# sloup/hessgpu

Hardware: AMD Instinct MI355X
Metric: Mpixels/s end-to-end (pyramid->descriptor), 1920x1080 (higher is better)
Workload: dtype f32; 1 GPU; 1920x1080 synthetic blobs (tests/fixtures.py), default octaves/DoG levels, top-K=4096 [configs[1]]; pipelined_contexts_per_gpu=6, streams_and_copier_threads_per_node=6, descriptor_order=pixel, distinct_images_per_gpu=8, input=u8 luminance resident in HBM; results delivered to host memory

## Files before the change

hessgpu_amd/csrc/k_feature.hip:

```cpp
#include <algorithm>
#include <cstdlib>
#include <type_traits>

#include "hess_dev.h"
#include "hess_devmath.h"

namespace hess {

namespace {

constexpr double kPI = 3.14159265358979323846;

__device__ __forceinline__ float rl(float v, int lane) {
  return __uint_as_float(__builtin_amdgcn_readlane(__float_as_uint(v), lane));
}
__device__ __forceinline__ int rli(int v, int lane) { return __builtin_amdgcn_readlane(v, lane); }

__device__ __forceinline__ void level_of(const Geom& g, int li, int* o, int* l) {
  *o = li / g.dog;
  *l = li - (*o) * g.dog + 1;
}


__device__ __forceinline__ int block_scan1(int a, int* total, int* lds) {
  const int lane = threadIdx.x & 63, wv = threadIdx.x >> 6, nw = blockDim.x >> 6;
  int ia = a;
#pragma unroll
  for (int d = 1; d < 64; d <<= 1) {
    int na = __shfl_up(ia, d);
    if (lane >= d) ia += na;
  }
  __syncthreads();
  if (lane == 63) lds[wv] = ia;
  __syncthreads();
  int oa = 0, sa = 0;
  for (int k = 0; k < nw; k++) {
    if (k < wv) oa += lds[k];
    sa += lds[k];
  }
  *total = sa;
  return oa + ia - a;
}

struct FeatScan {
  LimitParams lp;
  int multi;
  int* foffset;
  int* fsrc;
  int* feat_total;
  int* feat_first;
  int cap_feat;
  int* overflow;
  int* img_base;
  int* host_small;
};

__device__ __forceinline__ int wave_inclusive_scan(int v) {
  v += __builtin_amdgcn_update_dpp(0, v, 0x111 , 0xf, 0xf, true);
  v += __builtin_amdgcn_update_dpp(0, v, 0x112 , 0xf, 0xf, true);
  v += __builtin_amdgcn_update_dpp(0, v, 0x114 , 0xf, 0xf, true);
  v += __builtin_amdgcn_update_dpp(0, v, 0x118 , 0xf, 0xf, true);
  v += __builtin_amdgcn_update_dpp(0, v, 0x142 , 0xa, 0xf, false);
  v += __builtin_amdgcn_update_dpp(0, v, 0x143 , 0xc, 0xf, false);
  return v;
}

__device__ __forceinline__ void feature_scan_image(const Geom& g, const FeatScan& fs, const RawKey* list, const int* list_total,
                                                   int cap_list, const int* ocount, int b, int nimg, int chunk, int nchunk) {
  const LimitParams& lp = fs.lp;
  const int multi = fs.multi, cap_feat = fs.cap_feat;
  int* const foffset = fs.foffset; int* const fsrc = fs.fsrc; int* const feat_total = fs.feat_total;
  int* const feat_first = fs.feat_first; int* const overflow = fs.overflow; int* const img_base = fs.img_base;
  int* const host_small = fs.host_small;
  __shared__ int lds[64];
  __shared__ int lc[kMaxOct * kMaxDog];
  __shared__ int carry;
  const int tid = threadIdx.x, NTH = blockDim.x;
  const int n = list_total[b];
  const bool need_levels = multi && lp.threshold > 0 && lp.method != 3;
  if (need_levels) nchunk = 1;
  if (chunk >= nchunk) return;
  const int clen = (((n + nchunk - 1) / nchunk) + 1023) & ~1023;
  const int c0 = min(n, chunk * clen), c1 = min(n, c0 + clen);
  const int lane = tid & 63, wv = tid >> 6, nwv = NTH >> 6;
  for (int i = tid; i < g.nlev; i += NTH) lc[i] = 0;
  {
    int before = multi ? 0 : c0;
    if (multi && c0 > 0) {
      int part = 0;
      for (int k = tid; k < c0; k += NTH) part += ocount[(long long)b * cap_list + k];
      part = wave_inclusive_scan(part);
      if (lane == 63) lds[wv] = part;
      __syncthreads();
      for (int w = 0; w < nwv; w++) before += lds[w];
      __syncthreads();
    }
    if (tid == 0) carry = before;
  }
  __syncthreads();
  constexpr int FC = 16;
  for (int base = c0; base < c1; base += NTH * FC) {
    const int npass = min(c1 - base, NTH * FC);
    const int fc = (npass + NTH - 1) / NTH;
    int cc[FC], ex[FC], tot[FC], wsum = 0;
#pragma unroll
    for (int u = 0; u < FC; u++) {
      const int k = (wv * fc + u) * 64 + lane;
      const bool in = u < fc && k < npass;
      const long long at = (long long)b * cap_list + base + (in ? k : 0);
      cc[u] = in ? (multi ? ocount[at] : 1) : 0;
      const int inc = wave_inclusive_scan(cc[u]);
      ex[u] = inc - cc[u];
      tot[u] = __builtin_amdgcn_readlane(inc, 63);
      wsum += tot[u];
      if (need_levels && tot[u]) {
        const int lv = in ? list[at].level_index : 0;
        const int lv0 = __builtin_amdgcn_readfirstlane(lv);
        if (__builtin_amdgcn_ballot_w64(cc[u] != 0 && lv != lv0) == 0) {
          if (lane == 0) atomicAdd(&lc[lv0], tot[u]);
        } else if (cc[u]) {
          atomicAdd(&lc[lv], cc[u]);
        }
      }
    }
    if (lane == 0) lds[wv] = wsum;
    __syncthreads();
    int run = carry, ptot = 0;
    for (int w = 0; w < nwv; w++) {
      const int t = lds[w];
      run += w < wv ? t : 0;
      ptot += t;
    }
#pragma unroll
    for (int u = 0; u < FC; u++) {
      const int k = (wv * fc + u) * 64 + lane;
      if (u < fc && k < npass) {
        const int off = run + ex[u];
        foffset[(long long)b * cap_list + base + k] = off;
        for (int q = 0; q < cc[u]; q++)
          if (off + q < cap_feat) fsrc[(long long)b * cap_feat + off + q] = (base + k) * 4 + q;
      }
      run += tot[u];
    }
    __syncthreads();
    if (tid == 0) carry += ptot;
    __syncthreads();
  }
  if (chunk != nchunk - 1) return;
  if (tid == 0) {
    int total = carry, first = 0;
    if (multi && lp.threshold > 0 && lp.method != 3) {
      if (lp.method == 2) {
        int i = 0, nf = 0;
        for (; (nf < lp.threshold) && (i < g.nlev); ++i) nf += lc[i];
        if (nf < total) total = nf;
      } else {
        int i = 0;
        while (i < g.nlev && (total - lc[i]) > lp.threshold) { total -= lc[i]; first += lc[i]; i++; }
      }
    }
    if (first + total > cap_feat) { atomicMax(overflow + 1, first + total); total = cap_feat > first ? cap_feat - first : 0; }
    feat_total[b] = total;
    feat_first[b] = first;
    __threadfence();
    if (atomicAdd(overflow + 8, 1) == nimg - 1) {
      __threadfence();
      int acc = 0;
      for (int i = 0; i < nimg; i++) {
        img_base[i] = acc;
        if (host_small) host_small[i] = acc;
        acc += __hip_atomic_load(feat_total + i, __ATOMIC_RELAXED, __HIP_MEMORY_SCOPE_AGENT);
      }
      img_base[nimg] = acc;
      if (host_small) {
        host_small[nimg] = acc;
        for (int i = 0; i < 4; i++)
          host_small[nimg + 1 + i] = __hip_atomic_load(overflow + i, __ATOMIC_RELAXED, __HIP_MEMORY_SCOPE_AGENT);
      }
    }
  }
}

__global__ __launch_bounds__(1024) void feature_scan_kernel(Geom g, FeatScan fs, const RawKey* list, const int* list_total,
                                                            int cap_list, const int* ocount) {
  feature_scan_image(g, fs, list, list_total, cap_list, ocount, (int)blockIdx.y, (int)gridDim.y, (int)blockIdx.x, (int)gridDim.x);
}


__device__ __forceinline__ void key_range(const KeyBinJob& j, int b, int* first, int* count) {
  const int f = min(max(j.first_count[2 * b], 0), j.total);
  *first = f;
  *count = min(max(j.first_count[2 * b + 1], 0), min(j.max_count, j.total - f));
}

__device__ __forceinline__ int key_fixed(float v, int n) {
  const double d = (double)(v * (float)(1 << n)) + ((v >= 0.0) ? 0.5 : -0.5);
  return (d > -2147483649.0 && d < 2147483648.0) ? (int)d : (int)0x80000000u;
}

__global__ __launch_bounds__(256) void key_level_kernel(KeyBinJob j) {
  const int b = blockIdx.y, i = blockIdx.x * 256 + threadIdx.x;
  int first, count;
  key_range(j, b, &first, &count);
  if (i >= count) return;
  const HostKeypoint key = j.keys[first + i];
  const float s = j.rect ? (key.s < key.o ? key.s : key.o) / 12.0f : key.s;
  const int given = j.levels ? j.levels[i] : -1;
  int m = 0, hits = 0;
  for (int lv = 0; lv < j.nlev; lv++) {
    const KeyLevel t = j.table[lv];
    float sigmak = s;
    if (given >= 0) {
      if (given != lv) continue;
      sigmak = t.level_sigma;
    }
    if (((sigmak >= t.sigma_min) && (sigmak < t.sigma_max)) || ((sigmak < t.sigma_min) && lv == 0) ||
        ((sigmak > t.sigma_max) && lv == j.nlev - 1)) {
      if (hits < 2) {
        m |= (lv + 1) << (16 * hits);
        atomicAdd(j.level_count + b * j.nlev + lv, 1);
      }
      hits++;
    }
  }
  j.member[(long long)b * j.max_count + i] = m;
  if (hits > 2) atomicMax(j.overflow, j.cap_list + 1);
}

__global__ __launch_bounds__(64) void key_bin_kernel(KeyBinJob j) {
  const int lv = blockIdx.x, b = blockIdx.y, lane = threadIdx.x;
  int first, count;
  key_range(j, b, &first, &count);
  int off = 0;
  for (int l = lane; l < lv; l += 64) off += j.level_count[b * j.nlev + l];
  off = __builtin_amdgcn_readlane(wave_inclusive_scan(off), 63);
  const int* const member = j.member + (long long)b * j.max_count;
  constexpr int KU = 4;
  for (int base = 0; base < count; base += 64 * KU) {
    int m[KU];
#pragma unroll
    for (int u = 0; u < KU; u++) {
      const int i = base + u * 64 + lane;
      m[u] = i < count ? member[i] : 0;
    }
#pragma unroll
    for (int u = 0; u < KU; u++) {
      const bool hit = (m[u] & 0xFFFF) == lv + 1 || (m[u] >> 16) == lv + 1;
      const unsigned long long hits = __builtin_amdgcn_ballot_w64(hit);
      const int pos = off + __builtin_popcountll(hits & ((1ull << lane) - 1ull));
      if (hit && pos < j.cap_list) {
        const long long at = (long long)b * j.cap_list + pos;
        const RawKey rk = {lv, 0, 0, 0u, 0.0f, 0.0f, 0.0f, 0u};
        j.list[at] = rk;
        j.kmap[at] = base + u * 64 + lane;
        if (j.host_kmap) j.host_kmap[at] = base + u * 64 + lane;
      }
      off += __builtin_popcountll(hits);
    }
  }
  if (lv == j.nlev - 1 && lane == 0) {
    if (off > j.cap_list) { atomicMax(j.overflow, off); off = j.cap_list; }
    j.list_total[b] = off;
  }
}

__global__ __launch_bounds__(256) void key_record_kernel(KeyBinJob j) {
  const int b = blockIdx.y, pos = blockIdx.x * 256 + threadIdx.x;
  int first, count;
  key_range(j, b, &first, &count);
  if (pos >= min(j.list_total[b], j.cap_list)) return;
  const long long at = (long long)b * j.cap_list + pos;
  const int i = min(max(j.kmap[at], 0), count - 1), lv = min(max(j.list[at].level_index, 0), j.nlev - 1);
  const KeyLevel t = j.table[lv];
  const HostKeypoint key = j.keys[first + i];
  const float fX = (key.x - j.origin) / t.octave_sigma + 0.5f;
  const float fY = (key.y - j.origin) / t.octave_sigma + 0.5f;
  const float fScale = key.s / t.octave_sigma;
  const float fOrientation = j.rect ? key.o / t.octave_sigma : (float)fmod(2.0 * kPI - (double)key.o, 2.0 * kPI);
  FRec r;
  r.x = (uint32_t)key_fixed(fX, 10) & 0x00FFFFFFu;
  r.y = (uint32_t)key_fixed(fY, 10) & 0x00FFFFFFu;
  r.z = (uint32_t)key_fixed(fScale, 8) & 0x0000FFFFu;
  r.w = __float_as_uint(fOrientation);
  j.recs[at] = r;
}


__device__ __forceinline__ float dm_expf_inrange(float x) {
  float n = rintf(x * 1.44269504088896341f);
  float r = fmaf(n, -0.693359375f, x);
  r = fmaf(n, 2.12194440e-4f, r);
  float z = r * r;
  float p = 1.9875691500E-4f;
  p = fmaf(p, r, 1.3981999507E-3f);
  p = fmaf(p, r, 8.3334519073E-3f);
  p = fmaf(p, r, 4.1665795894E-2f);
  p = fmaf(p, r, 1.6666665459E-1f);
  p = fmaf(p, r, 5.0000001201E-1f);
  p = fmaf(p, z, r);
  p = p + 1.0f;
  return __builtin_amdgcn_ldexpf(p, (int)n);
}


__global__ __launch_bounds__(256) void orientation_kernel(Geom g, OrientParams op, const RawKey* list,
                                                          const int* list_total, int cap_list, const float* got,
                                                          FRec* recs, int* ocount) {
  __shared__ __attribute__((aligned(8))) float2 orec[4][66];
  const int lane = threadIdx.x & 63;
  float2* const myrec = orec[threadIdx.x >> 6];
  __shared__ int osize[4][36];
  int* const mysize = osize[threadIdx.x >> 6];
  const int b = blockIdx.y;
  const int n = list_total[b];
  const int nwaves = gridDim.x * 4;
  const float ten_degree_per_radius = 5.7295779513082320876798154814105f;
  const float radius_per_ten_degrees = (float)(1.0 / 5.7295779513082320876798154814105);
  const float one_third = (float)(1.0 / 3.0);

  for (int i = blockIdx.x * 4 + (threadIdx.x >> 6); i < n; i += nwaves) {
    const RawKey rk = list[(long long)b * cap_list + i];
    int o, l;
    level_of(g, rk.level_index, &o, &l);
    const OctGeom& og = g.o[o];
    const float2* gp = reinterpret_cast<const float2*>(got) + og.got_off + ((long long)(l - 1) * g.B + b) * og.plane;
    const int width = og.wa, height = og.h;

    float kx = rk.col + 0.5f, ky = rk.row + 0.5f, kz = op.level_sigma[l];
    FRec urec = {0u, 0u, 0u, 0u};
    if (op.existing) {
      urec = recs[(long long)b * cap_list + i];
      kx = (float)(urec.x & 0x00FFFFFFu) / 1024.0f;
      ky = (float)(urec.y & 0x00FFFFFFu) / 1024.0f;
      kz = (float)(urec.z & 0x0000FFFFu) / 256.0f;
    } else if (op.subpixel) {
      kx += rk.dx;
      ky += rk.dy;
      kz *= dm_powf_ln(op.ln_sigma_step, rk.ds);
    }
    uint32_t kw_bits = 0;
    int ocnt = 0;

    if (op.num_orientation != 0) {
      const float gsigma = kz * op.gaussian_factor;
      const float win = fabsf(kz) * op.sample_factor;
      const float dist_threshold = win * win + 0.5f;
      const float factor = -0.5f / (gsigma * gsigma);
      const float xmin = fmaxf(1.5f, floorf(kx - win) + 0.5f);
      const float ymin = fmaxf(1.5f, floorf(ky - win) + 0.5f);
      const float xmax = fminf(width - 1.5f, floorf(kx + win) + 0.5f);
      const float ymax = fminf(height - 1.5f, floorf(ky + win) + 0.5f);
      const int nxs = (xmax >= xmin) ? (int)(xmax - xmin) + 1 : 0;
      const int nys = (ymax >= ymin) ? (int)(ymax - ymin) + 1 : 0;
      const int total = nxs * nys;

      float vote = 0.0f;
      const float inv = 1.0f / (float)(nxs > 0 ? nxs : 1);
      const int base = (int)ymin * width + (int)xmin;
      for (int t0 = 0; t0 < total; t0 += 64) {
        const int t = t0 + lane;
        const int iy = (int)(((float)t + 0.5f) * inv);
        const int ix = t - __mul24(iy, nxs);
        const float x = xmin + (float)ix, y = ymin + (float)iy;
        float dy = y - ky;
        dy *= dy;
        const float dx = x - kx;
        const float sq_dist = fmaf(dx, dx, dy);
        const bool inside = (t < total) & !(sq_dist >= dist_threshold);
        const float2 gv = gp[inside ? base + __mul24(iy, width) + ix : 0];
        int bin = (int)floorf(gv.y * ten_degree_per_radius);
        bin = (bin < 0) ? bin + 36 : bin;
        const float e = dm_expf_inrange(sq_dist * factor);
        const bool counted = inside & ((unsigned)bin < 36u);
        const int key = counted ? bin : 63;
        uint32_t same_lo = ~0u, same_hi = ~0u;
#pragma unroll
        for (int k = 0; k < 6; k++) {
          const uint64_t bk = __builtin_amdgcn_ballot_w64((key >> k) & 1);
          const uint32_t km = (uint32_t)-((key >> k) & 1);
          same_lo &= ~((uint32_t)bk ^ km); same_hi &= ~((uint32_t)(bk >> 32) ^ km);
        }
        const int myrank = __builtin_amdgcn_mbcnt_hi(same_hi, __builtin_amdgcn_mbcnt_lo(same_lo, 0u));
        const int gsize = __popc(same_lo) + __popc(same_hi);
        if (lane < 36) mysize[lane] = 0;
        __builtin_amdgcn_wave_barrier();
        if (counted & (myrank + 1 == gsize)) mysize[bin] = gsize;
        __builtin_amdgcn_wave_barrier();
        const int mycnt = (lane < 36) ? mysize[lane] : 0;
        const int mystart = wave_inclusive_scan(mycnt) - mycnt;
        const int pos = __shfl(mystart, counted ? bin : 0) + myrank;
        __builtin_amdgcn_wave_barrier();
        if (counted) myrec[pos] = make_float2(gv.x, e);
        __builtin_amdgcn_wave_barrier();
        for (int k = 0; __builtin_amdgcn_ballot_w64(k < mycnt) != 0; k += 2) {
          if (k < mycnt) {
            const float2 r0 = myrec[mystart + k], r1 = myrec[mystart + k + 1];
            vote = fmaf(r0.x, r0.y, vote);
            if (k + 1 < mycnt) vote = fmaf(r1.x, r1.y, vote);
          }
        }
      }
      const int lp = (lane == 0) ? 35 : lane - 1;
      const int ln = (lane >= 35) ? 0 : lane + 1;
#pragma unroll
      for (int p = 0; p < 6; p++) {
        const float pre = __shfl(vote, lp), nxt = __shfl(vote, ln);
        vote = one_third * (pre + vote + nxt);
      }
      const float vote36 = rl(vote, 0);
      if (op.half_sift) {
        const float hi = __shfl(vote, (lane + 18) & 63);
        vote = (lane < 18) ? vote + hi : 0.0f;
      }
      if (lane >= 36) vote = -1.0f;
      float mx = vote;
#pragma unroll
      for (int d = 32; d >= 1; d >>= 1) mx = fmaxf(mx, __shfl_xor(mx, d));
      const float pre = __shfl(vote, lp);
      const float nxt_raw = __shfl(vote, ln);
      const float nxt = (lane == 35) ? vote36 : nxt_raw;

      if (op.num_orientation == 1 || op.existing) {
        const uint64_t mm = __ballot(lane < 36 && vote == mx);
        const int index_max = __builtin_ctzll(mm);
        const float p0 = rl(pre, index_max), n0 = rl(nxt, index_max), weight = mx;
        const float off = 0.5f * ((n0 - p0) / (weight + weight - n0 - p0));
        const float kw = radius_per_ten_degrees * ((float)index_max + 0.5f + off);
        kw_bits = __float_as_uint(kw);
      } else if (op.two_peaks) {
        const float vote_threshold = mx * 0.8f;
        const bool peak = (lane < 36) && (vote > vote_threshold) && (vote > pre) && (vote > nxt);
        const float di = 0.5f * ((nxt - pre) / (vote + vote - nxt - pre));
        const float rot = (float)lane + di + 0.5f;
        uint64_t pm = __ballot(peak);
        float mv0 = 0, mv1 = 0, mr0 = 0, mr1 = 0;
        int found = 0;
        while (pm) {
          const int j = __builtin_ctzll(pm);
          pm &= pm - 1;
          const float cw = rl(vote, j), cr = rl(rot, j);
          if (cw > mv1) {
            if (cw > mv0) { mv1 = mv0; mr1 = mr0; mv0 = cw; mr0 = cr; }
            else { mv1 = cw; mr1 = cr; }
            found++;
          }
        }
        float fr1 = mr0 / 36.0f;
        if (fr1 < 0) fr1 += 1.0f;
        const uint32_t us1 = (found == 0) ? 65535u : (uint32_t)(unsigned short)floorf(fr1 * 65535.0f);
        uint32_t us2 = 65535u;
        if (found > 1) {
          float fr2 = mr1 / 36.0f;
          if (fr2 < 0) fr2 += 1.0f;
          us2 = (uint32_t)(unsigned short)floorf(fr2 * 65535.0f);
        }
        kw_bits = (us2 << 16) | us1;
        ocnt = (us1 != 65535u) + (us2 != 65535u);
      } else {
        const float vote_threshold = mx * 0.8f;
        const bool peak = (lane < 36) && (vote > vote_threshold) && (vote > pre) && (vote > nxt);
        const float di = 0.5f * ((nxt - pre) / (vote + vote - nxt - pre));
        const float rot = (float)lane + di + 0.5f;
        uint64_t pm = __ballot(peak);
        float mv0 = 0, mv1 = 0, mv2 = 0, mv3 = 0, mr0 = 0, mr1 = 0, mr2 = 0, mr3 = 0;
        while (pm) {
          const int j = __builtin_ctzll(pm);
          pm &= pm - 1;
          float cw = rl(vote, j), cr = rl(rot, j);
          bool placed = false;
          float tw, tr;
#define HESS_INS(S, MV, MR)                                                     \
          if (S < ocnt) {                                                       \
            if (placed || MV < cw) { tw = MV; tr = MR; MV = cw; MR = cr; cw = tw; cr = tr; placed = true; } \
          } else if (S == ocnt) { MV = cw; MR = cr; }
          HESS_INS(0, mv0, mr0)
          HESS_INS(1, mv1, mr1)
          HESS_INS(2, mv2, mr2)
          HESS_INS(3, mv3, mr3)
#undef HESS_INS
          if (ocnt < 4) ocnt++;
        }
        const float mr[4] = {mr0, mr1, mr2, mr3};
        uint32_t packed = 0;
#pragma unroll
        for (int k = 0; k < 4; k++) {
          if (k < ocnt) {
            float orientation = mr[k] / 36.0f;
            if (orientation < 0) orientation += 1.0f;
            const uint32_t ui = (uint32_t)floorf(orientation * 255.0f);
            packed |= (ui << (8 * k));
          }
        }
        kw_bits = packed;
      }
    } else {
      kw_bits = __float_as_uint(0.0f);
    }
    if (lane == 0 && op.existing) {
      urec.w = kw_bits;
      recs[(long long)b * cap_list + i] = urec;
      ocount[(long long)b * cap_list + i] = 0;
    } else if (lane == 0) {
      uint32_t posX = (uint32_t)float_to_fixed(kx, 10) & 0x00FFFFFFu;
      uint32_t posY = (uint32_t)float_to_fixed(ky, 10) & 0x00FFFFFFu;
      posX |= (rk.packed & 0xFF000000u);
      posY |= ((rk.packed << 8) & 0xFF000000u);
      uint32_t scale = (uint32_t)float_to_fixed(kz, 8) & 0x0000FFFFu;
      scale |= ((rk.packed & 0x3u) << 30) | (((uint32_t)ocnt & 0x7u) << 27);
      FRec r;
      r.x = posX; r.y = posY; r.z = scale; r.w = kw_bits;
      recs[(long long)b * cap_list + i] = r;
      ocount[(long long)b * cap_list + i] = ocnt;
    }
  }
}


constexpr int DC_BINS = 12;
constexpr int DC_BIN_PITCH = 80;
constexpr int DC_ROWS = DC_BINS * DC_BIN_PITCH;

typedef const __attribute__((address_space(1))) char* GlobalBytes;
typedef float dfloat2 __attribute__((ext_vector_type(2)));

template <int N_>
struct DescChunk {
  static constexpr int N = N_;
  float nx[N_], ny[N_];
  float2 cc[N_];
  bool in[N_];
};

template <int S>
__device__ __forceinline__ void quad_fma(float& acc, float coef, float w) {
  static_assert(S >= 0 && S < 4, "quad lane");
  const float wb = __int_as_float(__builtin_amdgcn_mov_dpp(__float_as_int(w), S * 0x55, 0xF, 0xF, true));
  acc = fmaf(coef, wb, acc);
}


constexpr float rpi = (float)(4.0 / kPI);

__device__ __forceinline__ float record_pos(uint32_t xy) { return (float)(xy & 0x00FFFFFFu) / 1024.0f; }
__device__ __forceinline__ float record_scale(uint32_t z) { return (float)(z & 0x0000FFFFu) / 256.0f; }
__device__ __forceinline__ float multi_angle(int multi, uint32_t w, int k) {
  return multi == 2 ? (float)((2.0 * kPI / 65535.0) * (double)((w >> (16 * k)) & 0xFFFFu))
                    : (float)((2.0 * kPI / 255.0) * (double)((w >> (8 * k)) & 0xFFu));
}
__device__ __forceinline__ float record_angle(const DescParams& dp, uint32_t w, int k) {
  return dp.multi ? multi_angle(dp.multi, w, k) : __uint_as_float(w);
}

struct DescImage {
  int b, ftotal, ffirst;
  long long obase;
};
__device__ __forceinline__ DescImage desc_image(const DescParams& dp, const int* feat_total, const int* feat_first,
                                                const int* img_base) {
  DescImage im;
  im.b = blockIdx.y + dp.first_image;
  im.ftotal = feat_total[im.b];
  im.ffirst = feat_first[im.b];
  im.obase = img_base[im.b];
  if (dp.part_den > 1) {
    const int n = im.ftotal;
    const int lo = (int)((long long)n * dp.part / dp.part_den), hi = (int)((long long)n * (dp.part + 1) / dp.part_den);
    im.ffirst += lo; im.obase += lo; im.ftotal = hi - lo;
  }
  return im;
}

__device__ __forceinline__ int first_feature(const DescParams& dp, int wv) {
  int mw0 = blockIdx.x * 4 + wv;
  if (dp.xcd_block) {
    const int xcd = blockIdx.x & 7, wx = (int)(blockIdx.x >> 3) * 4 + wv;
    mw0 = ((wx / dp.xcd_block) * 8 + xcd) * dp.xcd_block + wx % dp.xcd_block;
  }
  return mw0;
}

__device__ __forceinline__ __amdgpu_buffer_rsrc_t plane_resource(const Geom& g, const OctGeom& og, const float* got, int l, int b) {
  const unsigned long long gpa = (unsigned long long)(reinterpret_cast<const float2*>(got) + og.got_off +
                                                      ((long long)(l - 1) * g.B + b) * og.plane);
  const GlobalBytes gp = (GlobalBytes)(
      ((unsigned long long)(unsigned)__builtin_amdgcn_readfirstlane((int)(gpa >> 32)) << 32) |
      (unsigned)__builtin_amdgcn_readfirstlane((int)(gpa & 0xFFFFFFFFull)));
  return __builtin_amdgcn_make_buffer_rsrc((void*)gp, 0, __builtin_amdgcn_readfirstlane(og.plane * 8),
                                           0x00020000 );
}

struct Feature {
  FRec rec;
  int k;
  int oidx;
  int width, height;
  __amdgpu_buffer_rsrc_t grsrc;
};
__device__ __forceinline__ Feature load_feature(const Geom& g, const DescImage& im, int m, const RawKey* list, int cap_list,
                                                const FRec* recs, const int* fsrc, int cap_feat, const float* got) {
  Feature f;
  const int src = fsrc[(long long)im.b * cap_feat + m];
  const int i = src >> 2;
  f.k = src & 3;
  f.oidx = m - im.ffirst;
  f.rec = recs[(long long)im.b * cap_list + i];
  const int li = list[(long long)im.b * cap_list + i].level_index;
  int o, l;
  level_of(g, li, &o, &l);
  const OctGeom& og = g.o[o];
  f.grsrc = plane_resource(g, og, got, l, im.b);
  f.width = og.wa;
  f.height = og.h;
  return f;
}

struct OrientedFrame {
  float kx, ky;
  float spt, anglef;
  float cspt, sspt;
  float crspt, srspt;
  float bsz;
};
__device__ __forceinline__ OrientedFrame oriented_frame(const DescParams& dp, const Feature& f) {
  OrientedFrame fr;
  fr.kx = record_pos(f.rec.x);
  fr.ky = record_pos(f.rec.y);
  const float kw = record_angle(dp, f.rec.w, f.k);
  fr.spt = fabsf(record_scale(f.rec.z) * dp.window_factor);
  float s, c;
  dm_sincosf(kw, &s, &c);
  fr.anglef = (kw > kPI) ? (float)(kw - (2.0 * kPI)) : kw;
  fr.cspt = c * fr.spt; fr.sspt = s * fr.spt;
  fr.crspt = c / fr.spt; fr.srspt = s / fr.spt;
  fr.bsz = fabsf(fr.cspt) + fabsf(fr.sspt);
  return fr;
}

__device__ __forceinline__ uint32_t theta_end(const DescParams& dp) { return dp.dynamic_indexing ? 0x41000001u : 0x41000000u; }

template <bool HOST_MIRROR>
__device__ __forceinline__ void keypoint_records(const DescParams& dp, uint32_t* const kst, const DescImage& im, const RawKey* list,
                                                 int cap_list, const FRec* recs, const int* fsrc, int cap_feat, HostKeypoint* keys) {
  for (int f0 = (gridDim.x - 1 - blockIdx.x) * 256; f0 < im.ftotal; f0 += gridDim.x * 256) {
    const int nrec = min(256, im.ftotal - f0);
    if ((int)threadIdx.x < nrec) {
      const int m = im.ffirst + f0 + threadIdx.x;
      const int src = fsrc[(long long)im.b * cap_feat + m];
      const int i = src >> 2, k = src & 3;
      const FRec rec = recs[(long long)im.b * cap_list + i];
      const int li = list[(long long)im.b * cap_list + i].level_index;
      const float kw = record_angle(dp, rec.w, k);
      const float kx = record_pos(rec.x), ky = record_pos(rec.y), kz = record_scale(rec.z);
      const float oss = dp.octave_sigma * (float)(1 << (li / dp.dog));
      const float offset = dp.lowe_origin ? 0.0f : 0.5f;
      HostKeypoint hk;
      hk.x = __fadd_rn(__fmul_rn(oss, kx - 0.5f), offset);
      hk.y = __fadd_rn(__fmul_rn(oss, ky - 0.5f), offset);
      hk.s = oss * kz;
      hk.o = (float)fmod(2.0 * kPI - (double)kw, 2.0 * kPI);
      hk.response = dm_h2f(((rec.x & 0xFF000000u) >> 16) | ((rec.y & 0xFF000000u) >> 24));
      hk.level = (uint16_t)li;
      hk.type = (uint16_t)((rec.z & 0xC0000000u) >> 30);
      *reinterpret_cast<HostKeypoint*>(kst + 6 * threadIdx.x) = hk;
    }
    __syncthreads();
    const uint2* const k2 = reinterpret_cast<const uint2*>(kst);
    uint2* const out = reinterpret_cast<uint2*>(keys + im.obase + f0);
    uint2* const hout = (HOST_MIRROR && dp.hkeys) ? reinterpret_cast<uint2*>(dp.hkeys + im.obase + f0) : nullptr;
    for (int j = threadIdx.x; j < 3 * nrec; j += 256) {
      const uint2 v = k2[j];
      out[j] = v;
      if (hout) hout[j] = v;
    }
    __syncthreads();
  }
}

__device__ __forceinline__ int unhoisted(int lane) {
  asm volatile("" : "+v"(lane));
  return lane;
}

__device__ __forceinline__ float* desc_at(void* base, long long o, int dim, bool u8) {
  return u8 ? reinterpret_cast<float*>(static_cast<char*>(base) + o * dim) : static_cast<float*>(base) + o * dim;
}

template <int N>
using DescValues = float __attribute__((ext_vector_type(N)));
template <bool HOST_MIRROR, int N>
__device__ __forceinline__ void finish_values(const DescParams& dp, bool u8, int lane, DescValues<N> v, float* dout, float* hout) {
  if (dp.normalize) {
#pragma unroll
    for (int pass = 0; pass < 2; pass++) {
      float part = v[0] * v[0];
#pragma unroll
      for (int i = 1; i < N; i++) part = fmaf(v[i], v[i], part);
#pragma unroll
      for (int d = 16; d >= 1; d >>= 1) part += __shfl_down(part, d);
      const float nrm = 1.0f / sqrtf(rl(part, 0));
#pragma unroll
      for (int i = 0; i < N; i++) v[i] = (pass == 0) ? fminf(0.2f, v[i] * nrm) : v[i] * nrm;
    }
  }
  if (u8) {
    if constexpr (N == 4) {
      const uint32_t q = desc_pack4(v[0], v[1], v[2], v[3]);
      const int at = 4 * unhoisted(lane);
      if (lane < 32) *reinterpret_cast<uint32_t*>(reinterpret_cast<char*>(dout) + at) = q;
      if (HOST_MIRROR && hout && lane < 32) *reinterpret_cast<uint32_t*>(reinterpret_cast<char*>(hout) + at) = q;
    } else {
      const uint32_t h = desc_byte(v[0]) | (desc_byte(v[1]) << 8);
      const uint32_t nb = (uint32_t)__builtin_amdgcn_mov_dpp((int)h, 0xF5 , 0xF, 0xF, true);
      const uint32_t q = h | (nb << 16);
      const int l = unhoisted(lane);
      const bool mine = l < 32 && !(l & 1);
      if (mine) *reinterpret_cast<uint32_t*>(reinterpret_cast<char*>(dout) + 2 * l) = q;
      if (HOST_MIRROR && hout && mine) *reinterpret_cast<uint32_t*>(reinterpret_cast<char*>(hout) + 2 * l) = q;
    }
    return;
  }
  if (lane < 32) *reinterpret_cast<DescValues<N>*>(dout + lane * N) = v;
  if (HOST_MIRROR && hout && lane < 32) *reinterpret_cast<DescValues<N>*>(hout + lane * N) = v;
}
template <int N>
__device__ __forceinline__ DescValues<N> staged_values(const float* staged, int lane) {
  DescValues<N> v = 0.0f;
  if (lane < 32) v = *reinterpret_cast<const DescValues<N>*>(staged + lane * N);
  return v;
}
template <bool HOST_MIRROR>
__device__ __forceinline__ void finish_descriptor(const DescParams& dp, bool u8, int lane, const float* staged, void* desc,
                                                  long long o) {
  const int dim = dp.half_sift ? 64 : 128;
  float* const dout = desc_at(desc, o, dim, u8);
  float* const hout = (HOST_MIRROR && dp.hdesc) ? desc_at(dp.hdesc, o, dim, u8) : nullptr;
  if (dp.half_sift) finish_values<HOST_MIRROR, 2>(dp, u8, lane, staged_values<2>(staged, lane), dout, hout);
  else finish_values<HOST_MIRROR, 4>(dp, u8, lane, staged_values<4>(staged, lane), dout, hout);
}

template <bool HOST_MIRROR, bool SEQ>
__global__ __launch_bounds__(256) void descriptor_kernel(Geom g, DescParams dp, const RawKey* list,
                                                         int cap_list, const FRec* recs,
                                                         const int* fsrc, const int* feat_total,
                                                         const int* feat_first, const int* img_base,
                                                         const float* got, HostKeypoint* keys, float* desc,
                                                         int cap_feat) {
  __shared__ __attribute__((aligned(16))) float dl[4][128];
  __shared__ __attribute__((aligned(16))) float crow[4][DC_ROWS];
  const int lane = threadIdx.x & 63, wv = threadIdx.x >> 6;
  const DescImage im = desc_image(dp, feat_total, feat_first, img_base);
  const int mycell = lane >> 2, sub = lane & 3;
  float* const rows = &crow[wv][0];

  static_assert(sizeof(HostKeypoint) == 24 && 4 * DC_ROWS * 4 >= 256 * 24, "record staging fits the table");
  keypoint_records<HOST_MIRROR>(dp, reinterpret_cast<uint32_t*>(&crow[0][0]), im, list, cap_list, recs, fsrc, cap_feat, keys);
  if (!desc) return;
  for (int i = lane; i < DC_ROWS; i += 64) rows[i] = 0.0f;
  float* const mycol = rows + mycell * 4 + sub;
  const float* const rdbin = rows + sub * DC_BIN_PITCH + mycell * 4;
  const uint32_t theta_end_bits = theta_end(dp);

  for (int mw = first_feature(dp, wv); mw < im.ftotal; mw += gridDim.x * 4) {
    const Feature f = load_feature(g, im, im.ffirst + im.ftotal - 1 - mw, list, cap_list, recs, fsrc, cap_feat, got);
    const OrientedFrame fr = oriented_frame(dp, f);
    const __amdgpu_buffer_rsrc_t grsrc = f.grsrc;
    const int width = f.width;
    const float crspt = fr.crspt, srspt = fr.srspt, anglef = fr.anglef;

    const float offx = (mycell & 3) - 1.5f, offy = (mycell >> 2) - 1.5f;
    const float ptx = fmaf(fr.cspt, offx, -(fr.sspt * offy)) + fr.kx;
    const float pty = fmaf(fr.cspt, offy, fr.sspt * offx) + fr.ky;
    const float xmin = fmaxf(1.5f, floorf(ptx - fr.bsz) + 0.5f);
    const float ymin = fmaxf(1.5f, floorf(pty - fr.bsz) + 0.5f);
    const float xmax = fminf(width - 1.5f, floorf(ptx + fr.bsz) + 0.5f);
    const float ymax = fminf(f.height - 1.5f, floorf(pty + fr.bsz) + 0.5f);
    const int nxs = (xmax >= xmin) ? (int)(xmax - xmin) + 1 : 0;
    const int nys = (ymax >= ymin) ? (int)(ymax - ymin) + 1 : 0;
    const int total = nxs * nys;
    int maxtotal = total;
#pragma unroll
    for (int d = 32; d >= 4; d >>= 1) maxtotal = max(maxtotal, __shfl_xor(maxtotal, d));
    maxtotal = rli(maxtotal, 0);
    const int nit = (maxtotal + 3) >> 2;
    const bool narrow = __any((nxs > 0) & (nxs < 4));
    const float fnxs = (float)nxs;
    const float inv = 1.0f / (float)(nxs > 0 ? nxs : 1);
    const int base = (int)ymin * width + (int)xmin;
    float xf = xmin + (float)sub;
    float yf = (total > 0) ? ymin : 3.0e38f;
    unsigned goff = (unsigned)(base + sub) * 8u;
    const float xwrap = xmax - 4.0f;
    const int rowskip = (width - nxs + 4) * 8;

    float acc0 = 0.0f, acc1 = 0.0f, acc2 = 0.0f;

    auto stage_a = [&](auto narrow_tag, int it0, auto& ck) {
      constexpr bool NARROW = decltype(narrow_tag)::value;
      constexpr int N = std::remove_reference_t<decltype(ck)>::N;
#pragma unroll
      for (int u = 0; u < N; u++) {
        if (NARROW) {
          const int t = (it0 + u) * 4 + sub;
          const int sy = (int)(((float)t + 0.5f) * inv);
          const int sx = t - __mul24(sy, nxs);
          xf = xmin + (float)sx;
          yf = (t < total) ? ymin + (float)sy : 3.0e38f;
          goff = (unsigned)(base + __mul24(sy, width) + sx) * 8u;
        }
        const float dx = xf - ptx, dy = yf - pty;
        ck.nx[u] = fmaf(crspt, dx, srspt * dy);
        ck.ny[u] = fmaf(crspt, dy, -(srspt * dx));
        ck.in[u] = (yf <= ymax) & (fabsf(ck.nx[u]) < 1.0f) & (fabsf(ck.ny[u]) < 1.0f);
        const dfloat2 gv = __builtin_amdgcn_raw_buffer_load_b64(grsrc, (int)(ck.in[u] ? goff : 0u), 0, 0);
        ck.cc[u] = make_float2(gv.x, gv.y);
        if (!NARROW) {
          const bool wrap = xf > xwrap;
          xf += wrap ? 4.0f - fnxs : 4.0f;
          yf += wrap ? 1.0f : 0.0f;
          goff += wrap ? (unsigned)rowskip : 32u;
        }
      }
    };
    auto accumulate = [&](const float4& c0, const float4& c1, const float4& c2, float wt) {
      quad_fma<0>(acc0, c0.x, wt); quad_fma<0>(acc1, c1.x, wt); quad_fma<0>(acc2, c2.x, wt);
      quad_fma<1>(acc0, c0.y, wt); quad_fma<1>(acc1, c1.y, wt); quad_fma<1>(acc2, c2.y, wt);
      quad_fma<2>(acc0, c0.z, wt); quad_fma<2>(acc1, c1.z, wt); quad_fma<2>(acc2, c2.z, wt);
      quad_fma<3>(acc0, c0.w, wt); quad_fma<3>(acc1, c1.w, wt); quad_fma<3>(acc2, c2.w, wt);
    };
    auto stage_b = [&](const auto& ck) {
      constexpr int N = std::remove_reference_t<decltype(ck)>::N;
      auto one = [&](int u) {
        const float nxn = fabsf(ck.nx[u]), nyn = fabsf(ck.ny[u]);
        const float dnx = ck.nx[u] + offx, dny = ck.ny[u] + offy;
        const float ww = dm_expf_inrange(-0.125f * fmaf(dnx, dnx, dny * dny));
        const float wx = 1.0f - nxn, wy = 1.0f - nyn;
        float wt = ww * wx * wy * ck.cc[u].x;
        float theta = (anglef - ck.cc[u].y) * rpi;
        theta = (theta < 0) ? theta + 8.0f : theta;
        const bool hit = ck.in[u] & (__float_as_uint(theta) < theta_end_bits);
        wt = hit ? wt : 0.0f;
        const float fo = floorf(theta);
        const float w1 = fo + 1.0f - theta, w2 = theta - fo;
        const int fidx = min(max((int)fo, 0), DC_BINS - 2);
        if (!SEQ) {
          float* const hp = rows + fidx * 64 + lane;
          const float a = hp[0], b2 = hp[64];
          hp[0] = fmaf(w1, wt, a);
          hp[64] = fmaf(w2, wt, b2);
          return;
        }
        mycol[fidx * DC_BIN_PITCH] = w1;
        mycol[fidx * DC_BIN_PITCH + DC_BIN_PITCH] = w2;
        __builtin_amdgcn_wave_barrier();
        const float4 c0 = *reinterpret_cast<const float4*>(rdbin);
        const float4 c1 = *reinterpret_cast<const float4*>(rdbin + 4 * DC_BIN_PITCH);
        const float4 c2 = *reinterpret_cast<const float4*>(rdbin + 8 * DC_BIN_PITCH);
        __builtin_amdgcn_wave_barrier();
        accumulate(c0, c1, c2, wt);
        mycol[fidx * DC_BIN_PITCH] = 0.0f;
        mycol[fidx * DC_BIN_PITCH + DC_BIN_PITCH] = 0.0f;
        __builtin_amdgcn_wave_barrier();
      };
#pragma unroll
      for (int u = 0; u < N; u++) {
        if (!__any(ck.in[u])) continue;
        one(u);
      }
    };
    if (narrow) {
      for (int it0 = 0; it0 < nit; it0++) {
        DescChunk<1> ck;
        stage_a(std::true_type{}, it0, ck);
        stage_b(ck);
      }
    } else {
      constexpr int UN = 4;
      DescChunk<UN> ca, cb;
      stage_a(std::false_type{}, 0, ca);
      for (int it0 = 0; it0 < nit; it0 += 2 * UN) {
        stage_a(std::false_type{}, it0 + UN, cb);
        stage_b(ca);
        if (it0 + UN >= nit) break;
        stage_a(std::false_type{}, it0 + 2 * UN, ca);
        stage_b(cb);
      }
    }
    if (!SEQ) {
      __builtin_amdgcn_wave_barrier();
      const float* const hb = rows + mycell * 4;
      const float4 h0 = *reinterpret_cast<const float4*>(hb + sub * 64);
      const float4 h1 = *reinterpret_cast<const float4*>(hb + (sub + 4) * 64);
      const float4 h2 = *reinterpret_cast<const float4*>(hb + (sub + 8) * 64);
      acc0 = (h0.x + h0.y) + (h0.z + h0.w);
      acc1 = (h1.x + h1.y) + (h1.z + h1.w);
      acc2 = (h2.x + h2.y) + (h2.z + h2.w);
      __builtin_amdgcn_wave_barrier();
      const float4 z4 = make_float4(0.f, 0.f, 0.f, 0.f);
      *reinterpret_cast<float4*>(rows + mycell * 4 + sub * 64) = z4;
      *reinterpret_cast<float4*>(rows + mycell * 4 + (sub + 4) * 64) = z4;
      *reinterpret_cast<float4*>(rows + mycell * 4 + (sub + 8) * 64) = z4;
      __builtin_amdgcn_wave_barrier();
    }
    if (sub == 0) acc0 += acc2;
    if (dp.half_sift) {
      dl[wv][mycell * 4 + sub] = acc0 + acc1;
    } else {
      dl[wv][mycell * 8 + sub] = acc0;
      dl[wv][mycell * 8 + 4 + sub] = acc1;
    }
    __builtin_amdgcn_wave_barrier();
    finish_descriptor<HOST_MIRROR>(dp, dp.u8 != 0, lane, dl[wv], desc, im.obase + f.oidx);
  }
}

#ifndef HESS_PX_COPIES
#define HESS_PX_COPIES 4
#endif
#ifndef HESS_PX_UNROLL
#define HESS_PX_UNROLL 2
#endif
constexpr int PX_COPIES = HESS_PX_COPIES;
constexpr int PX_COPY_U64 = 128 + 4;
constexpr int PX_WAVE_U64 = PX_COPIES * PX_COPY_U64;
#ifndef HESS_PX_WAVES
#define HESS_PX_WAVES 7
#endif
constexpr int PX_WAVES = HESS_PX_WAVES;
constexpr float PX_SPAN_EPS = 0.02f;
constexpr int PX_BAND_MAX = 4096;

template <int N_>
struct PixChunk {
  static constexpr int N = N_;
  float u[N_], v[N_];
  float2 cc[N_];
};

typedef __attribute__((address_space(3))) unsigned long long lds_u64;

#define HESS_PIXEL_KERNEL descriptor_pixel_kernel
#define HESS_PIXEL_U8 false
#include "k_feature_pixel.h"
#undef HESS_PIXEL_KERNEL
#undef HESS_PIXEL_U8
#define HESS_PIXEL_KERNEL descriptor_pixel_u8_kernel
#define HESS_PIXEL_U8 true
#include "k_feature_pixel.h"
#undef HESS_PIXEL_KERNEL
#undef HESS_PIXEL_U8

constexpr int RC_ROWS = 32;
constexpr int RC_WAVE = RC_ROWS * 64;
constexpr int RC_UNROLL = 4;

template <bool HOST_MIRROR>
__global__ __launch_bounds__(256) void descriptor_rect_kernel(Geom g, DescParams dp, const RawKey* list, int cap_list,
                                                              const FRec* recs, const int* fsrc, const int* feat_total,
                                                              const int* feat_first, const int* img_base, const float* got,
                                                              HostKeypoint* keys, float* desc, int cap_feat) {
  __shared__ __attribute__((aligned(16))) float dl[4][128];
  __shared__ __attribute__((aligned(16))) float hist[4][RC_WAVE];
  const int lane = threadIdx.x & 63, wv = threadIdx.x >> 6;
  const DescImage im = desc_image(dp, feat_total, feat_first, img_base);

  static_assert(sizeof(HostKeypoint) == 24 && 4 * RC_WAVE * 4 >= 256 * 24, "record staging fits the histograms");
  keypoint_records<HOST_MIRROR>(dp, reinterpret_cast<uint32_t*>(&hist[0][0]), im, list, cap_list, recs, fsrc, cap_feat, keys);
  if (!desc) return;
  float* const hw = &hist[wv][0];
  for (int i = lane; i < RC_WAVE; i += 64) hw[i] = 0.0f;
  float* const mine = hw + lane;
  const uint32_t theta_end_bits = theta_end(dp);

  for (int mw = first_feature(dp, wv); mw < im.ftotal; mw += gridDim.x * 4) {
    const Feature f = load_feature(g, im, im.ffirst + im.ftotal - 1 - mw, list, cap_list, recs, fsrc, cap_feat, got);
    const __amdgpu_buffer_rsrc_t grsrc = f.grsrc;
    const int width = f.width, height = f.height;
    const float kx = record_pos(f.rec.x), ky = record_pos(f.rec.y);
    const float sptx = record_scale(f.rec.z) * 0.25f, spty = __uint_as_float(f.rec.w) * 0.25f;

    float cx[4], bx0[4], bx1[4];
#pragma unroll
    for (int ix = 0; ix < 4; ix++) {
      cx[ix] = sptx * ((float)ix + 0.5f) + kx;
      bx0[ix] = fmaxf(1.5f, floorf(cx[ix] - sptx) + 0.5f);
      bx1[ix] = fminf((float)width - 1.5f, floorf(cx[ix] + sptx) + 0.5f);
    }
    const float xlo = fminf(fminf(bx0[0], bx0[1]), fminf(bx0[2], bx0[3]));
    const float xhi = fmaxf(fmaxf(bx1[0], bx1[1]), fmaxf(bx1[2], bx1[3]));
    const int ncols = (xhi >= xlo) ? (int)(xhi - xlo) + 1 : 0;

    for (int iy = 0; iy < 4; iy++) {
      const float cy = spty * ((float)iy + 0.5f) + ky;
      const float ymin = fmaxf(1.5f, floorf(cy - spty) + 0.5f);
      const float ymax = fminf((float)height - 1.5f, floorf(cy + spty) + 0.5f);
      const int nrows = (ymax >= ymin) ? (int)(ymax - ymin) + 1 : 0;
      for (int c0 = 0; c0 < ncols && nrows > 0; c0 += 64) {
        const int col = c0 + lane;
        const float x = xlo + (float)col;
        const bool xin = col < ncols;
        bool on[4];
        float wx[4];
        int non = 0;
#pragma unroll
        for (int ix = 0; ix < 4; ix++) {
          const float nx = (x - cx[ix]) / sptx;
          on[ix] = xin & (x >= bx0[ix]) & (x <= bx1[ix]) & (fabsf(nx) < 1.0f);
          wx[ix] = on[ix] ? 1.0f - fabsf(nx) : 0.0f;
          non += on[ix] ? 1 : 0;
        }
        float swx[4];
        int scol[4];
        {
          int ron = 0, roff = 0;
#pragma unroll
          for (int s = 0; s < 4; s++) { swx[s] = 0.0f; scol[s] = 0; }
#pragma unroll
          for (int ix = 0; ix < 4; ix++) {
            const int p = on[ix] ? ron : non + roff;
            ron += on[ix] ? 1 : 0;
            roff += on[ix] ? 0 : 1;
#pragma unroll
            for (int s = 0; s < 4; s++)
              if (p == s) { swx[s] = wx[ix]; scol[s] = ix * 8 * 64; }
          }
        }
        int nslot = non;
#pragma unroll
        for (int d = 32; d >= 1; d >>= 1) nslot = max(nslot, __shfl_xor(nslot, d));
        nslot = rli(nslot, 0);
        if (nslot == 0) continue;
        const unsigned coloff = (unsigned)((int)xlo + col) * 8u;

        for (int r0 = 0; r0 < nrows; r0 += RC_UNROLL) {
          float wy[RC_UNROLL];
          dfloat2 gv[RC_UNROLL];
#pragma unroll
          for (int u = 0; u < RC_UNROLL; u++) {
            const float y = ymin + (float)(r0 + u);
            const float ny = (y - cy) / spty;
            const bool live = (r0 + u < nrows) & (fabsf(ny) < 1.0f);
            wy[u] = live ? 1.0f - fabsf(ny) : 0.0f;
            const bool ld = live & (non > 0);
            const unsigned off = (unsigned)((int)y * width) * 8u + coloff;
            gv[u] = __builtin_amdgcn_raw_buffer_load_b64(grsrc, (int)(ld ? off : 0u), 0, 0);
          }
#pragma unroll
          for (int u = 0; u < RC_UNROLL; u++) {
            if (!(wy[u] > 0.0f)) continue;
            float t = (-gv[u].y) * rpi;
            t = (t < 0) ? t + 8.0f : t;
            t = (t == 0.0f) ? 0.0f : t;
            const bool hit = __float_as_uint(t) < theta_end_bits;
            float fo = floorf(t);
            float w1 = fo + 1.0f - t, w2 = t - fo;
            if (fo >= 8.0f) { fo = 7.0f; w1 = 0.0f; w2 = 1.0f; }
            if (!hit) { fo = 0.0f; w1 = 0.0f; w2 = 0.0f; }
            const int f0 = min(max((int)fo, 0), 7), f1 = (f0 + 1) & 7;
            const float mag = gv[u].x;
#pragma unroll
            for (int s = 0; s < 4; s++) {
              if (s >= nslot) break;
              const float wt = (s < non) ? (swx[s] * wy[u]) * mag : 0.0f;
              float* const h0 = mine + (scol[s] + f0 * 64);
              float* const h1 = mine + (scol[s] + f1 * 64);
              const float a0 = *h0, a1 = *h1;
              *h0 = fmaf(w1, wt, a0);
              *h1 = fmaf(w2, wt, a1);
            }
          }
        }
      }
      __builtin_amdgcn_wave_barrier();
      const int r = lane & 31, hh = lane >> 5;
      float part = 0.0f;
#pragma unroll 8
      for (int k = 0; k < 32; k++) part += hw[r * 64 + 32 * hh + ((k + r) & 31)];
      const float tot = part + __shfl_down(part, 32);
      __builtin_amdgcn_wave_barrier();
      const float4 z4 = make_float4(0.f, 0.f, 0.f, 0.f);
#pragma unroll
      for (int k = 0; k < RC_WAVE / 256; k++) *reinterpret_cast<float4*>(hw + (k * 64 + lane) * 4) = z4;
      const float fold = tot + __shfl_down(tot, 4);
      const int ix = r >> 3, bin = r & 7;
      if (dp.half_sift) {
        if (lane < 32 && bin < 4) dl[wv][(iy * 4 + ix) * 4 + bin] = fold;
      } else if (lane < 32) {
        dl[wv][(iy * 4 + ix) * 8 + bin] = tot;
      }
      __builtin_amdgcn_wave_barrier();
    }
    finish_descriptor<HOST_MIRROR>(dp, dp.u8 != 0, lane, dl[wv], desc, im.obase + f.oidx);
  }
}

}

void launch_key_bin(hipStream_t st, const KeyBinJob& job, int batch) {
  if (job.max_count > 0)
    hipLaunchKernelGGL(key_level_kernel, dim3((job.max_count + 255) / 256, batch), dim3(256), 0, st, job);
  hipLaunchKernelGGL(key_bin_kernel, dim3(job.nlev, batch), dim3(64), 0, st, job);
  if (job.max_count > 0)
    hipLaunchKernelGGL(key_record_kernel, dim3((job.cap_list + 255) / 256, batch), dim3(256), 0, st, job);
}

void launch_orientation(hipStream_t st, const Geom& g, const OrientParams& op, const FeatureBuffers& fb, const float* got,
                        int batch) {
  int blocks = (fb.cap_list + 3) / 4;
  if (blocks > 2048) blocks = 2048;
  if (blocks < 1) blocks = 1;
  hipLaunchKernelGGL(orientation_kernel, dim3(blocks, batch), dim3(256), 0, st, g, op, fb.list, fb.list_total, fb.cap_list,
                     got, fb.recs, fb.ocount);
}

void launch_feature_scan(hipStream_t st, const Geom& g, const LimitParams& lp, int multi, const FeatureBuffers& fb,
                         int* overflow, int* host_small, int batch) {
  FeatScan fs;
  fs.lp = lp; fs.multi = multi; fs.foffset = fb.foffset; fs.fsrc = fb.fsrc; fs.feat_total = fb.feat_total;
  fs.feat_first = fb.feat_first; fs.cap_feat = fb.cap_feat; fs.overflow = overflow; fs.img_base = fb.img_base;
  fs.host_small = host_small;
  const int nchunk = std::min(16, std::max(1, fb.cap_list / 4096));
  hipLaunchKernelGGL(feature_scan_kernel, dim3(nchunk, batch), dim3(1024), 0, st, g, fs, fb.list, fb.list_total, fb.cap_list,
                     fb.ocount);
}

using DescKernel = void (*)(Geom, DescParams, const RawKey*, int, const FRec*, const int*, const int*, const int*, const int*,
                            const float*, HostKeypoint*, float*, int);
static DescKernel descriptor_kernel_for(bool rect, bool pixel, bool u8, bool sequential, bool mirror) {
  if (rect) return mirror ? descriptor_rect_kernel<true> : descriptor_rect_kernel<false>;
  if (pixel && u8) return mirror ? descriptor_pixel_u8_kernel<true> : descriptor_pixel_u8_kernel<false>;
  if (pixel) return mirror ? descriptor_pixel_kernel<true> : descriptor_pixel_kernel<false>;
  if (sequential) return mirror ? descriptor_kernel<true, true> : descriptor_kernel<false, true>;
  return mirror ? descriptor_kernel<true, false> : descriptor_kernel<false, false>;
}

void launch_descriptor(hipStream_t st, const Geom& g, const DescParams& dp, const FeatureBuffers& fb, const float* got,
                       int batch, int seen_features) {
  const int den = dp.part_den > 1 ? dp.part_den : 1;
  int blocks = 2048;
  if (seen_features > 0) {
    const long long want = ((long long)seen_features * 5 / 4 / den + 3) / 4;
    blocks = (int)std::min<long long>(16384, std::max<long long>(256, (want + 127) / 128 * 128));
  }
  const int cap_blocks = (fb.cap_feat / den + 3) / 4;
  if (blocks > cap_blocks) blocks = cap_blocks;
  if (blocks < 1) blocks = 1;
  DescParams dpx = dp;
  dpx.px_band = std::min(PX_BAND_MAX, std::max(64, dp.px_band > 0 ? dp.px_band : PX_BAND_MAX));
  if (dp.rect || (dpx.xcd_block && ((blocks * 4) % (8 * dpx.xcd_block) != 0 || blocks % 8 != 0))) dpx.xcd_block = 0;
  hipLaunchKernelGGL(descriptor_kernel_for(dp.rect, dp.pixel, dp.u8, dp.sequential, dp.hkeys || dp.hdesc), dim3(blocks, batch),
                     dim3(256), 0, st, g, dpx, fb.list, fb.cap_list, fb.recs, fb.fsrc, fb.feat_total, fb.feat_first, fb.img_base,
                     got, fb.keys, fb.desc, fb.cap_feat);
}

}
```

Measured before the change: 23330 Mpix/s.

## Iterate only pixels inside the circular window in orientation voting

The orientation kernel no longer walks the full bounding square of the sample window. For each band of rows it computes the per-row x-span inside the circle, prefix-scans the span lengths, and stores row descriptors in LDS. Lanes then map linear indices to rows through a start-bitmask and mbcnt, so the corner pixels outside the circle are never visited. This cuts the iterations of the per-64-sample histogram loop by roughly the circle-to-square area ratio, in exchange for extra per-band setup with a scan, LDS atomics and barriers, plus a small epsilon and slack in the span bounds that could change edge inclusion.

```diff
diff --git a/hessgpu_amd/csrc/k_feature.hip b/hessgpu_amd/csrc/k_feature.hip
--- a/hessgpu_amd/csrc/k_feature.hip
+++ b/hessgpu_amd/csrc/k_feature.hip
@@ -302,6 +302,8 @@
   return __builtin_amdgcn_ldexpf(p, (int)n);
 }
 
+constexpr float ORI_SPAN_EPS = 0.02f;
+constexpr float ORI_SPAN_SLACK = 1.0e-6f;
 
 __global__ __launch_bounds__(256) void orientation_kernel(Geom g, OrientParams op, const RawKey* list,
                                                           const int* list_total, int cap_list, const float* got,
@@ -309,6 +311,10 @@
   __shared__ __attribute__((aligned(8))) float2 orec[4][66];
   const int lane = threadIdx.x & 63;
   float2* const myrec = orec[threadIdx.x >> 6];
+  __shared__ unsigned long long ostarts[4][64];
+  __shared__ __attribute__((aligned(16))) uint4 orows[4][64];
+  unsigned long long* const mystarts = ostarts[threadIdx.x >> 6];
+  uint4* const myrows = orows[threadIdx.x >> 6];
   __shared__ int osize[4][36];
   int* const mysize = osize[threadIdx.x >> 6];
   const int b = blockIdx.y;
@@ -352,22 +358,62 @@
       const float ymax = fminf(height - 1.5f, floorf(ky + win) + 0.5f);
       const int nxs = (xmax >= xmin) ? (int)(xmax - xmin) + 1 : 0;
       const int nys = (ymax >= ymin) ? (int)(ymax - ymin) + 1 : 0;
-      const int total = nxs * nys;
 
       float vote = 0.0f;
-      const float inv = 1.0f / (float)(nxs > 0 ? nxs : 1);
       const int base = (int)ymin * width + (int)xmin;
-      for (int t0 = 0; t0 < total; t0 += 64) {
+      const int nxs_u = __builtin_amdgcn_readfirstlane(nxs), nys_u = __builtin_amdgcn_readfirstlane(nys);
+      const int band_rows = (nxs_u <= 64) ? 64 : max(1, 64 >> min(31, 26 - __builtin_clz(nxs_u - 1)));
+      const float span_off = kx - xmin;
+      const float span_slack = dist_threshold * ORI_SPAN_SLACK;
+      for (int jb = 0; jb < nys_u; jb += band_rows) {
+      const int nrow = min(band_rows, nys_u - jb);
+      int T;
+      uint32_t mword_lo, mword_hi;
+      {
+        const float yrow = ymin + (float)(jb + lane);
+        float dyr = yrow - ky;
+        dyr *= dyr;
+        const float rem = (dist_threshold - dyr) + span_slack;
+        const float hw = __builtin_amdgcn_sqrtf(fmaxf(rem, 0.0f)) + ORI_SPAN_EPS;
+        const float flo = fmaxf(ceilf(span_off - hw), 0.0f), fhi = fminf(floorf(span_off + hw), (float)(nxs_u - 1));
+        const int len = (lane < nrow && rem >= 0.0f && fhi >= flo) ? (int)(fhi - flo) + 1 : 0;
+        const int ilo = (int)flo;
+        const int incl = wave_inclusive_scan(len);
+        const int S = incl - len;
+        T = __builtin_amdgcn_readlane(incl, 63);
+        const uint64_t ne = __builtin_amdgcn_ballot_w64(len > 0);
+        const int r = (int)__builtin_amdgcn_mbcnt_hi((uint32_t)(ne >> 32), __builtin_amdgcn_mbcnt_lo((uint32_t)ne, 0u));
+        __builtin_amdgcn_wave_barrier();
+        mystarts[lane] = 0ull;
+        __builtin_amdgcn_wave_barrier();
+        if (len > 0) {
+          (void)__hip_atomic_fetch_or(mystarts + (S >> 6), 1ull << (S & 63), __ATOMIC_RELAXED, __HIP_MEMORY_SCOPE_WORKGROUP);
+          myrows[r] = make_uint4((uint32_t)(base + (jb + lane) * width + ilo - S), __float_as_uint(xmin + (float)(ilo - S)),
+                                 __float_as_uint(yrow), 0u);
+        }
+        __builtin_amdgcn_wave_barrier();
+        const unsigned long long mw = mystarts[lane];
+        mword_lo = (uint32_t)mw; mword_hi = (uint32_t)(mw >> 32);
+      }
+      int rows_before = -1;
+      for (int t0 = 0; t0 < T; t0 += 64) {
         const int t = t0 + lane;
-        const int iy = (int)(((float)t + 0.5f) * inv);
-        const int ix = t - __mul24(iy, nxs);
-        const float x = xmin + (float)ix, y = ymin + (float)iy;
+        const int sw = min(t0 >> 6, 63);
+        const uint32_t mlo = (uint32_t)__builtin_amdgcn_readlane((int)mword_lo, sw), mhi = (uint32_t)__builtin_amdgcn_readlane((int)mword_hi, sw);
+        const uint64_t m64 = ((uint64_t)mhi << 32) | mlo;
+        int rr = rows_before + (int)__builtin_amdgcn_mbcnt_hi(mhi, __builtin_amdgcn_mbcnt_lo(mlo, 0u)) + (__builtin_amdgcn_inverse_ballot_w64(m64) ? 1 : 0);
+        rows_before += __builtin_popcountll(m64);
+        rr = (int)min((unsigned)rr, 63u);
+        const uint4 re = myrows[rr];
+        const float x = __uint_as_float(re.y) + (float)t, y = __uint_as_float(re.z);
+        const int gidx = (int)re.x + t;
+        const bool in_seq = t < T;
         float dy = y - ky;
         dy *= dy;
         const float dx = x - kx;
         const float sq_dist = fmaf(dx, dx, dy);
-        const bool inside = (t < total) & !(sq_dist >= dist_threshold);
-        const float2 gv = gp[inside ? base + __mul24(iy, width) + ix : 0];
+        const bool inside = in_seq & !(sq_dist >= dist_threshold);
+        const float2 gv = gp[inside ? gidx : 0];
         int bin = (int)floorf(gv.y * ten_degree_per_radius);
         bin = (bin < 0) ? bin + 36 : bin;
         const float e = dm_expf_inrange(sq_dist * factor);
@@ -399,6 +445,7 @@
             if (k + 1 < mycnt) vote = fmaf(r1.x, r1.y, vote);
           }
         }
+      }
       }
       const int lp = (lane == 0) ? 35 : lane - 1;
       const int ln = (lane >= 35) ? 0 : lane + 1;
```

New measurement: 23540 Mpix/s, median of 6. About the same (+0.9%).
